# mozack/vdjer

Hardware: NVIDIA B200
Metric: graph_build_prune_windows_per_sec (higher is better)
Workload: dtype u8/u64

## Files before the change

### vdjer_b200/csrc/kernels.cuh

```cuda
#pragma once
#include <cstdint>
#include <cuda_runtime.h>

namespace vdjg {

typedef unsigned long long u64;
typedef unsigned int u32;
typedef unsigned short u16;
typedef unsigned char u8;

constexpr u64 EMPTY64 = ~0ull;
constexpr u64 INF64 = ~0ull;
constexpr u32 NIL32 = 0xFFFFFFFFu;
constexpr u32 CNT_CAP = 32765;
constexpr int GATE_Q = 20;
constexpr int HIQ = 30;
constexpr int FLB = 6;
constexpr u32 CNT2_MASK = 0x00FFFFFFu;
constexpr int CNT2_IN = 24;
constexpr u64 LOG_A = 1ull << 62, LOG_B = 1ull << 63;
constexpr int QSUM_SAT = 214;
constexpr int MAX_LOG_RANKS = 11;
constexpr u32 CNT_MULTI = 0x80000000u;
constexpr u32 CNT_SURV = 0x40000000u;
// ... 294 lines not shown
            if (rev && code < 4) code = 3u - code;
            const u8 q = (u8)(rec[1 + g.L + sj] - '!');
            a.qual[r * (u64)g.L + j] = q;
            okq = q >= GATE_Q;
            hiq = q >= HIQ;
        }
        const u32 b0 = __ballot_sync(0xFFFFFFFFu, code < 4 && (code & 1u));
        const u32 b1 = __ballot_sync(0xFFFFFFFFu, code < 4 && (code & 2u));
        const u32 bv = __ballot_sync(0xFFFFFFFFu, code < 4);
        const u32 bg = __ballot_sync(0xFFFFFFFFu, code < 4 && okq);
        const u32 bh = __ballot_sync(0xFFFFFFFFu, code < 4 && hiq);
        const u32 be = __ballot_sync(0xFFFFFFFFu, code == 5);
        if (lane == 0) {
            if (be) atomicMin(&a.bad[1], r);
            a.bases[r * (u64)g.nb + (j0 >> 5)] = spread_bits(b0) | (spread_bits(b1) << 1);
            if (j0 & 32) {
                a.valid[r * (u64)g.nm + (j0 >> 6)] = vword | ((u64)bv << 32);
                a.good[r * (u64)g.nm + (j0 >> 6)] = gword | ((u64)bg << 32);
                a.hiq[r * (u64)g.nm + (j0 >> 6)] = hword | ((u64)bh << 32);
            } else {
                vword = bv; gword = bg; hword = bh;
                if (j0 + 32 >= g.L) {
                    a.valid[r * (u64)g.nm + (j0 >> 6)] = vword;
                    a.good[r * (u64)g.nm + (j0 >> 6)] = gword;
                    a.hiq[r * (u64)g.nm + (j0 >> 6)] = hword;
                }
            }
        }
    }
}
__global__ void __launch_bounds__(THREADS)
k_pack(PackArgs a, Geom g) {
    const u32 lane = threadIdx.x & 31;
    const u64 warp = ((u64)blockIdx.x * THREADS + threadIdx.x) >> 5, n_warps = ((u64)gridDim.x * THREADS) >> 5;
    const u64 rec_len = 2ull * g.L + 1;
    for (u64 i = warp; i < a.n; i += n_warps) {
        const unsigned char *rec = a.text + i * rec_len;
        if (!a.fwd_only) {
            pack_record(a, g, rec, a.r0 + i, false, lane);
        } else {
            pack_record(a, g, rec, a.r0 + 2 * i, false, lane);
            pack_record(a, g, rec, a.r0 + 2 * i + 1, true, lane);
        }
    }
}

struct BlockTiles {
    u64 *buf;
    u64 *bar;
    u32 words, off_b, off_c, off_d;
    __device__ __forceinline__ const u64 *a(int i) const { return buf + i * words; }
    __device__ __forceinline__ const u64 *b(int i) const { return buf + i * words + off_b; }
    __device__ __forceinline__ const u64 *c(int i) const { return buf + i * words + off_c; }
    __device__ __forceinline__ const u64 *d(int i) const { return buf + i * words + off_d; }
};
__host__ __device__ inline size_t block_tile_bytes(const Geom &g, int n_masks) {
    return (size_t)2 * g.tile_rec * (size_t)(g.nb + n_masks * g.nm) * 8 + 16;
}
__device__ __forceinline__ BlockTiles tiles_setup(unsigned char *smem, const Geom &g, int n_masks) {
    BlockTiles t;
    t.words = g.tile_rec * (u32)(g.nb + n_masks * g.nm);
    t.off_b = g.tile_rec * (u32)g.nb;
    t.off_c = t.off_b + g.tile_rec * (u32)g.nm;
    t.off_d = t.off_c + g.tile_rec * (u32)g.nm;
    t.buf = reinterpret_cast<u64 *>(smem);
    t.bar = t.buf + 2 * t.words;
    if (threadIdx.x == 0) {
        mbar_init(&t.bar[0], 1);
        mbar_init(&t.bar[1], 1);
        fence_mbar_init();
        fence_proxy_async();
    }
    __syncthreads();
    return t;
}
__device__ __forceinline__ void tiles_issue(const BlockTiles &t, int i, const Geom &g, u64 tile,
                                            const u64 *ga, const u64 *gb, const u64 *gc, const u64 *gd = nullptr) {
    const u32 bytes_a = g.tile_rec * (u32)g.nb * 8u, bytes_m = g.tile_rec * (u32)g.nm * 8u;
    u64 *dst = t.buf + i * t.words;
    mbar_expect_tx(&t.bar[i], bytes_a + (gd ? 3 : 2) * bytes_m);
    tma_load_1d(dst, ga + tile * g.tile_rec * (u64)g.nb, bytes_a, &t.bar[i]);
    tma_load_1d(dst + t.off_b, gb + tile * g.tile_rec * (u64)g.nm, bytes_m, &t.bar[i]);
    tma_load_1d(dst + t.off_c, gc + tile * g.tile_rec * (u64)g.nm, bytes_m, &t.bar[i]);
    if (gd) tma_load_1d(dst + t.off_d, gd + tile * g.tile_rec * (u64)g.nm, bytes_m, &t.bar[i]);
}

__device__ __forceinline__ void extract_bits128(const u64 *m, int nw, int bit0, u64 &lo, u64 &hi) {
    const int wi = bit0 >> 6, sh = bit0 & 63;
    const u64 w0 = wi < nw ? m[wi] : 0ull;
    const u64 w1 = wi + 1 < nw ? m[wi + 1] : 0ull;
    const u64 w2 = wi + 2 < nw ? m[wi + 2] : 0ull;
    if (sh) { lo = (w0 >> sh) | (w1 << (64 - sh)); hi = (w1 >> sh) | (w2 << (64 - sh)); }
    else { lo = w0; hi = w1; }
}
__device__ __forceinline__ void shr128(u64 &lo, u64 &hi, int s) {
    if (s >= 64) { lo = hi >> (s - 64); hi = 0ull; }
    else if (s) { lo = (lo >> s) | (hi << (64 - s)); hi >>= s; }
}
__device__ __forceinline__ u64 erode128(u64 lo, u64 hi, int k) {
    u64 pl = lo, ph = hi, al = ~0ull, ah = ~0ull;
    int alen = 0;
    for (int plen = 1; plen <= k; plen <<= 1) {
        if (k & plen) {
            u64 tl = pl, th = ph;
            shr128(tl, th, alen);
            al &= tl; ah &= th;
            alen += plen;
        }
        u64 tl = pl, th = ph;
        shr128(tl, th, plen);
        pl &= tl; ph &= th;
    }
    return al;
}
__device__ __forceinline__ u64 erode64(u64 m, int k) {
    u64 p = m, a = ~0ull;
    int alen = 0;
    for (int plen = 1; plen <= k; plen <<= 1) {
        if (k & plen) { a &= p >> alen; alen += plen; }
        p &= p >> plen;
    }
    return a;
}
__device__ __forceinline__ u64 window_mask(const u64 *m, int nw, int i0, const Geom &g) {
    u64 lo, hi;
    extract_bits128(m, nw, i0, lo, hi);
    return g.seg + g.k <= 64 ? erode64(lo, g.k) : erode128(lo, hi, g.k);
}

struct Mini {
    u32 *buf;
    u32 x, pre;
    int r;
    __device__ __forceinline__ void sweep(int span) {
        u32 run = ~0u;
        for (int j = span - 1; j >= 0; j--) { run = min(run, buf[j * THREADS]); buf[j * THREADS] = run; }
    }
    __device__ __forceinline__ u32 start(u64 lo, u64 hi, const Geom &g) {
        for (int j = 0; j < g.span; j++) {
            x = (u32)lo & g.mmask;
            buf[j * THREADS] = mini_hash(x);
            lo = (lo >> 2) | (hi << 62);
            hi >>= 2;
        }
        sweep(g.span);
        r = 0; pre = ~0u;
        return buf[0];
    }
    __device__ __forceinline__ u32 step(u32 c, const Geom &g) {
        x = (x >> 2) | (c << (2 * (g.m - 1)));
        const u32 h = mini_hash(x);
        buf[r * THREADS] = h;
        r++;
        if (r == g.span) { sweep(g.span); r = 0; pre = ~0u; return buf[0]; }
        pre = min(pre, h);
        return min(buf[r * THREADS], pre);
    }
};

struct SegRuns {
    u64 V, G, H;
    u32 starts;
    u32 left;
    u32 ord;
    __device__ __forceinline__ bool next(int n, int &s, int &len) {
        if (!left) return false;
        s = __ffs((int)left) - 1;
        left &= left - 1;
        const u64 stop = ((((u64)starts | ~V) >> s) >> 1) | (1ull << (n - s - 1));
        len = __ffsll((long long)stop);
        ord++;
        return true;
    }
    __device__ __forceinline__ u32 has_next(int s, int len) const { return (u32)(V >> (s + len)) & 1u; }
};
template <bool KMERS, class OnGated>
__device__ __forceinline__ SegRuns scan_runs(const u64 *sb, const u64 *sg, const u64 *sv, const u64 *sh, u32 rec, int i0, int n,
                                             const Geom &g, u32 *scratch, u8 *sbk, OnGated on_gated) {
    Mini mn;
    mn.buf = scratch;
    SegRuns sr;
    sr.V = sr.G = sr.H = 0; sr.starts = 0; sr.ord = 0;
    u64 lo = 0, hi = 0, nbase = 0;
    if (n > 0) {
        sr.V = window_mask(sv + (size_t)rec * g.nm, g.nm, i0, g);
        sr.G = window_mask(sg + (size_t)rec * g.nm, g.nm, i0, g);
        if (sh) sr.H = window_mask(sh + (size_t)rec * g.nm, g.nm, i0, g);
        const u64 *b = sb + (size_t)rec * g.nb;
        extract_kmer(b, g.nb, i0, g.kmask_lo, g.kmask_hi, lo, hi);
        const int j = i0 + g.k;
        u64 nl = 0, nh;
        if (j < 32 * g.nb) extract_kmer(b, g.nb, j, ~0ull, 0ull, nl, nh);
        nbase = nl;
    }
    u32 run_len = 0, run_b = 0, minh = 0, n_starts = 0;
    for (int j = 0; j < g.seg; j++) {
        if (j < n) {
            if (j == 0) minh = mn.start(lo, hi, g);
            else {
                const u32 c = (u32)nbase & 3u;
                nbase >>= 2;
                minh = mn.step(c, g);
                if (KMERS) kmer_succ(lo, hi, c, g.k, lo, hi);
            }
            const bool v = (sr.V >> j) & 1ull;
            const u32 b = mini_bucket(minh);
            const bool fresh = v && (run_len == 0 || b != run_b || run_len == (u32)g.run_max);
            if (fresh) {
                sbk[n_starts * THREADS] = (u8)b;
                n_starts++;
                sr.starts |= 1u << j;
                run_b = b;
                run_len = 0;
            }
            run_len = v ? run_len + 1 : 0;
            if (KMERS && ((sr.G >> j) & 1ull)) on_gated(lo, hi, b);
        }
    }
    sr.left = sr.starts;
    return sr;
}

__host__ __device__ inline size_t align128(size_t x) { return (x + 127) & ~(size_t)127; }
__host__ __device__ inline size_t count_head_bytes() {
    return ((size_t)NBUCKET * BHLL / 4 + (size_t)3 * NBUCKET) * sizeof(u32);
}
__host__ __device__ inline size_t scratch_bytes(const Geom &g) { return (size_t)g.span * THREADS * sizeof(u32); }
__host__ __device__ inline size_t sbk_bytes(const Geom &g) { return align128((size_t)g.seg * THREADS); }
__device__ __forceinline__ void byte_max(u32 *words, u32 idx, u32 v, bool global) {
    u32 *wp = words + (idx >> 2);
    const u32 sh = (idx & 3u) * 8u;
    u32 cur = *reinterpret_cast<volatile u32 *>(wp);
    while (((cur >> sh) & 0xFFu) < v) {
        const u32 nv = (cur & ~(0xFFu << sh)) | (v << sh);
        const u32 old = atomicCAS(wp, cur, nv);
        if (old == cur) break;
        cur = old;
    }
}
__global__ void __launch_bounds__(THREADS)
k_count(const u64 *__restrict__ bases, const u64 *__restrict__ good, const u64 *__restrict__ valid,
        Geom g, u64 tile0, u64 tile1 , u32 *hll, u64 *hist ) {
    extern __shared__ __align__(128) unsigned char smem[];
    constexpr int HW = NBUCKET * BHLL / 4;
    u32 *reg = reinterpret_cast<u32 *>(smem);
    u32 *sh = reg + HW;
    for (int i = threadIdx.x; i < HW + 3 * NBUCKET; i += THREADS) reg[i] = 0;
    u32 *scratch = reinterpret_cast<u32 *>(smem + count_head_bytes()) + threadIdx.x;
    u8 *sbk = smem + count_head_bytes() + scratch_bytes(g) + threadIdx.x;
    BlockTiles t = tiles_setup(smem + count_head_bytes() + scratch_bytes(g) + sbk_bytes(g), g, 2);
    const u32 rec = threadIdx.x / (u32)g.segs, i0 = (threadIdx.x % (u32)g.segs) * (u32)g.seg;
    const int n = rec < g.tile_rec ? max(0, min(g.seg, g.w - (int)i0)) : 0;
    const u64 n_iter = (tile1 - tile0 + gridDim.x - 1) / gridDim.x;
    if (threadIdx.x == 0 && tile0 + blockIdx.x < tile1) tiles_issue(t, 0, g, tile0 + blockIdx.x, bases, good, valid);
    u64 tile = tile0 + blockIdx.x;
    for (u64 it = 0; it < n_iter; it++, tile += gridDim.x) {
        const int buf = (int)(it & 1);
        if (tile < tile1) {
            if (threadIdx.x == 0 && tile + gridDim.x < tile1) tiles_issue(t, buf ^ 1, g, tile + gridDim.x, bases, good, valid);
            mbar_wait(&t.bar[buf], (u32)(it >> 1) & 1);
            SegRuns sr = scan_runs<true>(t.a(buf), t.b(buf), t.c(buf), nullptr, rec, (int)i0, n, g, scratch, sbk,
                [&](u64 lo, u64 hi, u32 b) {
                    const u64 h = hash_key(lo, hi);
                    byte_max(reg, b * BHLL + ((u32)h & (BHLL - 1)), (u32)__clzll((long long)(h >> BHLL_BITS)) - (BHLL_BITS - 1), false);
                });
            int rs, len;
            while (sr.next(n, rs, len)) {
                const u32 b = sbk[(sr.ord - 1) * THREADS], gm = (u32)(sr.G >> rs) & ((1u << len) - 1u);
                atomicAdd(&sh[b], 1u);
                if (gm) atomicAdd(&sh[NBUCKET + b], (u32)__popc(gm));
                atomicAdd(&sh[2 * NBUCKET + b], (u32)len);
            }
        }
        __syncthreads();
        if ((it & 0xFFFF) == 0xFFFF) {
            for (int i = threadIdx.x; i < 3 * NBUCKET; i += THREADS) { u32 v = sh[i]; if (v) { atomicAdd(&hist[i], (u64)v); sh[i] = 0; } }
            __syncthreads();
        }
    }
    for (int i = threadIdx.x; i < HW; i += THREADS) {
        const u32 v = reg[i];
        for (int b = 0; v && b < 4; b++) if ((v >> (8 * b)) & 0xFFu) byte_max(hll, 4u * i + b, (v >> (8 * b)) & 0xFFu, true);
    }
    for (int i = threadIdx.x; i < 3 * NBUCKET; i += THREADS)
        if (sh[i]) atomicAdd(&hist[i], (u64)sh[i]);
}

constexpr int RUN_WORDS = 4;
constexpr int RUN_FP_BITS = 22;
__device__ __forceinline__ u32 run_len(u64 w2) { return ((u32)(w2 >> 48) & 31u) + 1u; }
__device__ __forceinline__ u32 run_bucket(u64 w3) { return (u32)(w3 >> STAMP_BITS) & (NBUCKET - 1); }
__device__ __forceinline__ void ld_run(const u64 *p, u64 &a, u64 &b, u64 &c, u64 &d) {
    asm volatile("ld.global.cs.v4.b64 {%0,%1,%2,%3}, [%4];" : "=l"(a), "=l"(b), "=l"(c), "=l"(d) : "l"(p) : "memory");
}

struct ScatterArgs {
    const u64 *bases, *good, *valid, *hiq;
    u64 *const *tbase;
    u64 *cursor;
    const u64 *limit;
    u64 rec_base;
    Counters *ctr;
};
struct ScatterSmem {
    u32 *cnt;
    u32 *fill;
    u32 *boff;
    u64 *gbase;
    u64 **dst;
    u32 *fp;
    u32 *n_list;
    u8 *sbk;
    u64 *list;
    u64 *stage;
    unsigned char *tiles;
};
__host__ __device__ inline size_t scatter_carve(ScatterSmem *o, unsigned char *base, const Geom &g) {
    size_t off = 0;
    auto take = [&](size_t bytes) { size_t at = off; off = align128(off + bytes); return at; };
    const size_t a_cnt = take((size_t)NBUCKET * 4), a_fill = take((size_t)NBUCKET * 4), a_boff = take((size_t)(NBUCKET + 1) * 4), a_gbase = take((size_t)NBUCKET * 8);
    const size_t a_dst = take((size_t)NBUCKET * 8), a_fp = take((size_t)g.tile_rec * 4), a_n = take(16);
    const size_t a_list = take((size_t)g.stage_runs * 16), a_sbk = take(sbk_bytes(g));
    const size_t stage_b = (size_t)g.stage_runs * RUN_WORDS * 8, scr_b = scratch_bytes(g);
    const size_t a_stage = take(stage_b > scr_b ? stage_b : scr_b), a_tiles = take(block_tile_bytes(g, 3));
    if (o) {
        o->cnt = reinterpret_cast<u32 *>(base + a_cnt); o->fill = reinterpret_cast<u32 *>(base + a_fill); o->boff = reinterpret_cast<u32 *>(base + a_boff);
        o->gbase = reinterpret_cast<u64 *>(base + a_gbase); o->dst = reinterpret_cast<u64 **>(base + a_dst);
        o->fp = reinterpret_cast<u32 *>(base + a_fp); o->n_list = reinterpret_cast<u32 *>(base + a_n);
        o->sbk = base + a_sbk;
        o->list = reinterpret_cast<u64 *>(base + a_list); o->stage = reinterpret_cast<u64 *>(base + a_stage);
        o->tiles = base + a_tiles;
    }
    return off;
}
__device__ __forceinline__ void build_run(u64 d0, u64 d1, const u64 *sb, const u64 *sv, const u32 *sfp, const Geom &g, u64 rec0,
                                          u64 &w0, u64 &w1, u64 &w2, u64 &w3) {
    const u32 rec = (u32)d1 & 0xFFFFu, a = (u32)(d1 >> 16) & 0xFFu, b = (u32)(d1 >> 24) & 0xFFu;
    extract_kmer(sb + (size_t)rec * g.nb, g.nb, (int)a, ~0ull, ~0ull, w0, w1);
    const u32 f = sfp[rec], fp = f & ((1u << RUN_FP_BITS) - 1);
    u64 prev = 0;
    if (a > 0 && bit_at(sv + (size_t)rec * g.nm, (int)a - 1)) prev = 1ull | ((u64)base_at(sb + (size_t)rec * g.nb, (int)a - 1) << 1);
    w2 = d0 | ((u64)(f >> 31) << 54) | (prev << 55) | ((u64)(fp >> 16) << 58);
    w3 = ((rec0 + rec) * (u64)g.w + a) | ((u64)b << STAMP_BITS) | ((u64)(fp & 0xFFFFu) << 48);
}

__global__ void __launch_bounds__(THREADS)
k_scatter(ScatterArgs a, Geom g, Part pt) {
    extern __shared__ __align__(128) unsigned char smem[];
    const int NU = NBUCKET >> pt.ushift;
    ScatterSmem sm;
    scatter_carve(&sm, smem, g);
    BlockTiles t = tiles_setup(sm.tiles, g, 3);
    const u32 lane = threadIdx.x & 31, wid = threadIdx.x >> 5;
    u32 *scratch = reinterpret_cast<u32 *>(sm.stage) + threadIdx.x;
    const u32 rec = threadIdx.x / (u32)g.segs, i0 = (threadIdx.x % (u32)g.segs) * (u32)g.seg;
    const int n = rec < g.tile_rec ? max(0, min(g.seg, g.w - (int)i0)) : 0;
    const u64 n_iter = (g.n_tiles + gridDim.x - 1) / gridDim.x;
    for (int u = threadIdx.x; u < NU; u += THREADS) sm.dst[u] = a.tbase[u];
    if (threadIdx.x == 0 && blockIdx.x < g.n_tiles) tiles_issue(t, 0, g, blockIdx.x, a.bases, a.good, a.valid, a.hiq);
    u64 tile = blockIdx.x;
    for (u64 it = 0; it < n_iter; it++, tile += gridDim.x) {
        const int buf = (int)(it & 1);
        if (tile >= g.n_tiles) break;
        for (int i = threadIdx.x; i < NU; i += THREADS) { sm.cnt[i] = 0; sm.fill[i] = 0; }
        if (threadIdx.x == 0) {
            *sm.n_list = 0;
            if (tile + gridDim.x < g.n_tiles) tiles_issue(t, buf ^ 1, g, tile + gridDim.x, a.bases, a.good, a.valid, a.hiq);
        }
        mbar_wait(&t.bar[buf], (u32)(it >> 1) & 1);
        __syncthreads();
        const u64 *sb = t.a(buf), *sg = t.b(buf), *sv = t.c(buf), *sh = t.d(buf);
        const u64 rec0 = a.rec_base + tile * g.tile_rec;
        for (u32 r = threadIdx.x; r < g.tile_rec; r += THREADS) {
            u64 h = 0x9E3779B97F4A7C15ull;
            for (int i = 0; i < g.nb; i++) h = hash_key(sb[(size_t)r * g.nb + i], h);
            for (int i = 0; i < g.nm; i++) h = hash_key(sv[(size_t)r * g.nm + i], h);
            const u32 rec_hi = (extract_mask(sh + (size_t)r * g.nm, g.nm, 0) & g.kones) == g.kones ? 1u : 0u;
            sm.fp[r] = ((u32)(h >> 32) & ((1u << RUN_FP_BITS) - 1)) | (rec_hi << 31);
        }
        __syncthreads();
        {
            SegRuns sr = scan_runs<false>(sb, sg, sv, sh, rec, (int)i0, n, g, scratch, sm.sbk + threadIdx.x, [](u64, u64, u32) {});
            for (;;) {
                int rs = 0, len = 1;
                const bool has = sr.next(n, rs, len);
                if (!__ballot_sync(0xFFFFFFFFu, has)) break;
                const u32 b = has ? sm.sbk[(sr.ord - 1) * THREADS + threadIdx.x] : 0u, u = b >> pt.ushift;
                const bool ship = has && sm.dst[u];
                const u32 ball = __ballot_sync(0xFFFFFFFFu, ship);
                if (!ball) continue;
                u32 e0 = 0;
                if (lane == 0) e0 = atomicAdd(sm.n_list, (u32)__popc(ball));
                e0 = __shfl_sync(0xFFFFFFFFu, e0, 0);
                if (ship) {
                    const u32 lm = (1u << len) - 1u;
                    const u64 d0 = (u64)((u32)(sr.G >> rs) & lm) | ((u64)((u32)(sr.H >> rs) & lm) << 24) | ((u64)(len - 1) << 48) |
                                   ((u64)sr.has_next(rs, len) << 53);
                    const u64 d1 = (u64)rec | ((u64)(i0 + rs) << 16) | ((u64)b << 24);
                    const u32 e = e0 + (u32)__popc(ball & ((1u << lane) - 1u));
                    if (e < g.stage_runs) {
                        sm.list[2 * e] = d0; sm.list[2 * e + 1] = d1;
                        atomicAdd(&sm.cnt[u], 1u);
                    } else {
                        u64 w0, w1, w2, w3;
                        build_run(d0, d1, sb, sv, sm.fp, g, rec0, w0, w1, w2, w3);
                        const u64 at = atomicAdd(&a.cursor[u], 1ull);
                        if (at < a.limit[u]) st_sector(sm.dst[u] + at * RUN_WORDS, w0, w1, w2, w3);
                        else atomicExch(&a.ctr->overflow, 4u);
                    }
                }
            }
        }
        __syncthreads();
        for (int u = threadIdx.x; u < NU; u += THREADS) {
            const u32 c = sm.cnt[u];
            u64 gbs = INF64;
            if (c) {
                gbs = atomicAdd(&a.cursor[u], (u64)c);
                if (gbs + c > a.limit[u]) { atomicExch(&a.ctr->overflow, 4u); gbs = INF64; }
            }
            sm.gbase[u] = gbs;
        }
        if (wid == 0) {
            const int per = (NU + 31) / 32;
            u32 sum = 0;
            for (int j = 0; j < per; j++) { int u = lane * per + j; if (u < NU) sum += sm.cnt[u]; }
            u32 incl = sum;
            for (int o = 1; o < 32; o <<= 1) { u32 v = __shfl_up_sync(0xFFFFFFFFu, incl, o); if ((int)lane >= o) incl += v; }
            u32 run = incl - sum;
            for (int j = 0; j < per; j++) {
                int u = lane * per + j;
                if (u < NU) { sm.boff[u] = run; run += sm.cnt[u]; }
            }
            if (lane == 31) sm.boff[NU] = run;
        }
        __syncthreads();
        const u32 n_list = min(*sm.n_list, g.stage_runs);
        for (u32 e = threadIdx.x; e < n_list; e += THREADS) {
            const u64 d0 = sm.list[2 * e], d1 = sm.list[2 * e + 1];
            const u32 u = ((u32)(d1 >> 24) & 0xFFu) >> pt.ushift;
            u64 w0, w1, w2, w3;
            build_run(d0, d1, sb, sv, sm.fp, g, rec0, w0, w1, w2, w3);
            u64 *dst = sm.stage + (size_t)(sm.boff[u] + atomicAdd(&sm.fill[u], 1u)) * RUN_WORDS;
            dst[0] = w0; dst[1] = w1; dst[2] = w2; dst[3] = w3;
        }
        fence_proxy_async();
        __syncthreads();
        for (int u = threadIdx.x; u < NU; u += THREADS) {
            const u32 c = sm.boff[u + 1] - sm.boff[u];
            const u64 gbs = sm.gbase[u];
            if (c && gbs != INF64) tma_store_1d(sm.dst[u] + gbs * RUN_WORDS, sm.stage + (size_t)sm.boff[u] * RUN_WORDS, c * (u32)(RUN_WORDS * 8));
        }
        tma_store_commit();
        tma_store_wait_read();
        __syncthreads();
    }
}

__global__ void k_init_table1(Slot1 *t, u64 cap) {
    u64 i = (u64)blockIdx.x * blockDim.x + threadIdx.x, stride = (u64)gridDim.x * blockDim.x;
    for (; i < cap; i += stride)
        st_sector(&t[i], EMPTY64, EMPTY64, (u64)0 | ((u64)NIL32 << 32), (u64)NIL32);
}
__global__ void k_init_table2(Slot2 *t, u64 cap) {
    u64 i = (u64)blockIdx.x * blockDim.x + threadIdx.x, stride = (u64)gridDim.x * blockDim.x;
    for (; i < cap; i += stride) {
        st_sector(&t[i], EMPTY64, EMPTY64, (u64)0 | ((u64)NIL32 << 32), INF64);
        st_sector(reinterpret_cast<char *>(&t[i]) + 32, INF64, INF64, INF64, INF64);
    }
}

__device__ __noinline__ bool same_words(const u64 *b1, const u64 *b2, int nb, const u64 *v1, const u64 *v2, int nm) {
    u64 diff = 0;
    for (int i = 0; i < nb; i++) diff |= b1[i] ^ b2[i];
    for (int i = 0; i < nm; i++) diff |= v1[i] ^ v2[i];
    return diff == 0;
}
__device__ __forceinline__ bool same_read(const Reads &rd, u64 r1, u64 r2, int nb, int nm) {
    const int d1 = rd.dev_of(r1), d2 = rd.dev_of(r2);
    const u64 l1 = r1 - rd.rec_base[d1], l2 = r2 - rd.rec_base[d2];
    if (rd.any_strand && rd.strand[d1][l1] != rd.strand[d2][l2]) return false;
    return same_words(rd.bases[d1] + l1 * nb, rd.bases[d2] + l2 * nb, nb, rd.valid[d1] + l1 * nm, rd.valid[d2] + l2 * nm, nm);
}

struct Pass1Args {
    const u64 *runs;
    Reads rd;
    Slot1 *table;
    u64 cap;
    u64 *log;
    u32 log_blocks;
    u32 nb_ranks;
    Counters *ctr;
};

constexpr u32 QFLUSH = 96;
constexpr u32 QCAP = 32 * BATCH + QFLUSH;
constexpr u32 QDENSE = 20;
constexpr int HOTC_BITS = 6;
constexpr u32 HOTC = 1u << HOTC_BITS;
constexpr u32 QFLUSH1 = 32;
constexpr u32 QCAP1 = 32 * BATCH + QFLUSH1;
template <bool WIDE, u32 QC = QCAP>
struct WarpQueue {
    u64 *lo, *w1, *w2;
    u32 *idx;
    __device__ __forceinline__ void setup(unsigned char *smem) {
        unsigned char *p = smem + (threadIdx.x >> 5) * bytes();
        lo = reinterpret_cast<u64 *>(p);
        w1 = lo + QC;
        w2 = w1 + QC;
        idx = reinterpret_cast<u32 *>(w1 + (WIDE ? 2 : 1) * QC);
    }
    __host__ __device__ static constexpr size_t bytes() { return (size_t)QC * (WIDE ? 28 : 20); }
    template <class Make>
    __device__ __forceinline__ u32 push_lazy(u32 qn, bool defer, u64 l, u32 i, Make make) {
        const u32 lane = threadIdx.x & 31;
        const u32 ballot = __ballot_sync(0xFFFFFFFFu, defer);
        if (defer) {
            const u32 pos = qn + __popc(ballot & ((1u << lane) - 1));
            u64 a, b;
            make(a, b);
            lo[pos] = l; w1[pos] = a; idx[pos] = i;
            if (WIDE) w2[pos] = b;
        }
        return qn + __popc(ballot);
    }
    __device__ __forceinline__ u32 push(u32 qn, bool defer, u64 l, u64 a, u64 b, u32 i) {
        const u32 lane = threadIdx.x & 31;
        const u32 ballot = __ballot_sync(0xFFFFFFFFu, defer);
        if (defer) {
            const u32 pos = qn + __popc(ballot & ((1u << lane) - 1));
            lo[pos] = l; w1[pos] = a; idx[pos] = i;
            if (WIDE) w2[pos] = b;
        }
        return qn + __popc(ballot);
    }
};

struct RunCursor {
    u64 w0, w1, w2;
    u64 stamp0;
    u32 off, len;
    u32 l;
    u32 j;
    u32 rem;
};
struct RunFeed {
    u64 *rw;
    u32 cnt, incl, total;
    u32 live;
    template <bool GATED_ONLY>
    __device__ __forceinline__ static u32 selected(u64 w2) {
        return GATED_ONLY ? (u32)w2 & 0xFFFFFFu : (1u << run_len(w2)) - 1u;
    }
    template <bool GATED_ONLY>
    __device__ __forceinline__ void load(const u64 *runs, u64 ri, u64 n_runs) {
        const u32 lane = threadIdx.x & 31;
        u64 w0 = 0, w1 = 0, w2 = 0, w3 = 0;
        cnt = 0;
        if (ri < n_runs) {
            ld_run(runs + ri * RUN_WORDS, w0, w1, w2, w3);
            cnt = (u32)__popc(selected<GATED_ONLY>(w2));
        }
        incl = cnt;
        for (int o = 1; o < 32; o <<= 1) { const u32 v = __shfl_up_sync(0xFFFFFFFFu, incl, o); if ((int)lane >= o) incl += v; }
        total = __shfl_sync(0xFFFFFFFFu, incl, 31);
        live = __ballot_sync(0xFFFFFFFFu, cnt != 0);
        __syncwarp();
        u64 *p = rw + lane * RUN_WORDS;
        p[0] = w0; p[1] = w1; p[2] = ri < n_runs ? w2 : 0ull; p[3] = w3;
        __syncwarp();
    }
    template <bool TAB2>
    __device__ __forceinline__ void open(RunCursor &c, const Part &pt) const {
        const u64 *p = rw + c.l * RUN_WORDS;
        c.w0 = p[0]; c.w1 = p[1]; c.w2 = p[2];
        const u64 w3 = p[3];
        c.stamp0 = w3 & ((1ull << STAMP_BITS) - 1);
        const uint4 ut = __ldg(reinterpret_cast<const uint4 *>(pt.ut + (run_bucket(w3) >> pt.ushift)));
        c.off = TAB2 ? ut.z : ut.x;
        c.len = TAB2 ? ut.w : ut.y;
    }
    template <bool GATED_ONLY, bool TAB2>
    __device__ __forceinline__ void seek(u32 t, RunCursor &c, const Part &pt) const {
        u32 l = 0;
#pragma unroll
        for (int s = 16; s; s >>= 1) { const u32 v = __shfl_sync(0xFFFFFFFFu, incl, l + s - 1); if (v <= t) l += s; }
        u32 nth = t - __shfl_sync(0xFFFFFFFFu, incl - cnt, l);
        c.l = l;
        open<TAB2>(c, pt);
        u32 m = selected<GATED_ONLY>(c.w2), j = 0;
        if (GATED_ONLY) {
#pragma unroll
            for (int s = 16; s; s >>= 1) {
                const u32 k = (u32)__popc(m & ((1u << s) - 1u));
                if (nth >= k) { nth -= k; m >>= s; j += s; }
            }
            m >>= 1;
        } else {
            j = nth;
            m >>= j + 1;
        }
        c.j = j; c.rem = m;
    }
    __device__ __forceinline__ u32 fingerprint(u32 l, const Part &pt) const {
        const u64 *p = rw + l * RUN_WORDS;
        return (((u32)(p[3] >> 48) & 0xFFFFu) | (((u32)(p[2] >> 58) & 0x3Fu) << 16)) & (u32)((1ull << pt.fb) - 1);
    }
    template <bool GATED_ONLY, bool TAB2>
    __device__ __forceinline__ void next(RunCursor &c, const Part &pt) const {
        if (c.rem) {
            const u32 s = (u32)__ffs((int)c.rem);
            c.j += s; c.rem >>= s;
            return;
        }
        const u32 ahead = c.l < 31 ? live >> (c.l + 1) : 0u;
        c.l += ahead ? (u32)__ffs((int)ahead) : 0u;
        open<TAB2>(c, pt);
        const u32 m = selected<GATED_ONLY>(c.w2);
        const u32 s = m ? (u32)__ffs((int)m) : 1u;
        c.j = s - 1; c.rem = m >> s;
    }
};
__device__ __forceinline__ void run_kmer(const Geom &g, const RunCursor &c, u64 &lo, u64 &hi, u32 &idx) {
    const u32 sh = 2u * c.j;
    lo = sh ? (c.w0 >> sh) | (c.w1 << (64 - sh)) : c.w0;
    hi = c.w1 >> sh;
    lo &= g.kmask_lo; hi &= g.kmask_hi;
    idx = slot_in(hash_slot(lo, hi), c.off, c.len);
}
__device__ __forceinline__ u32 run_flags(const Geom &g, u64 w0, u64 w1, u64 w2, u32 j) {
    const u32 p = j + (u32)g.k;
    const u32 nb = (u32)((p < 32 ? w0 >> (2 * p) : w1 >> (2 * (p - 32)))) & 3u;
    const bool has_next = j + 1 < run_len(w2) || ((w2 >> 53) & 1ull);
    return (has_next ? 1u | (nb << 1) : 0u) | ((u32)(w2 >> (24 + j)) & 1u) << 3 | ((u32)(w2 >> 54) & 1u) << 4;
}
__device__ __forceinline__ u32 run_flags2(const Geom &g, u64 w0, u64 w1, u64 w2, u32 j) {
    const u32 p = j + (u32)g.k;
    const u32 nb = (u32)((p < 32 ? w0 >> (2 * p) : w1 >> (2 * (p - 32)))) & 3u;
    const bool has_next = j + 1 < run_len(w2) || ((w2 >> 53) & 1ull);
    const u32 prev = j ? 1u | (((u32)(w0 >> (2 * (j - 1))) & 3u) << 1) : (u32)(w2 >> 55) & 7u;
    return (has_next ? 1u | (nb << 1) : 0u) | prev << 3;
}
template <bool WIDE>
__device__ __forceinline__ void pack_tuple(const Part &pt, u64 hi, u32 fl, u32 fp, u64 stamp, u64 &t1, u64 &t2) {
    t1 = hi | ((u64)fl << pt.hb) | ((u64)fp << (pt.hb + FLB));
    if (WIDE) t2 = stamp;
    else { t1 |= stamp << (pt.hb + FLB + pt.fb); t2 = 0; }
}

struct LogCursor { u32 base, used; };

template <bool WIDE>
__device__ __forceinline__ u32 pass1_drain(const Pass1Args &a, const Geom &g, const Part &pt, WarpQueue<WIDE, QCAP1> &q,
                                           u32 qn, LogCursor &lc, bool final) {
    const u32 lane = threadIdx.x & 31, lt = (1u << lane) - 1;
    u32 next = 0;
    bool have = false;
    u64 lo = 0, hi = 0, stamp = 0, rw1 = 0, rw2 = 0;
    u32 idx = 0, probe = 0, fp = 0, fl = 0;
    __syncwarp();
    for (;;) {
        const u32 need = __ballot_sync(0xFFFFFFFFu, !have);
        const u32 avail = qn - next;
        if (avail == 0 && (need == 0xFFFFFFFFu || (!final && 32 - __popc(need) < (int)pt.qdense1))) break;
        if (need && avail) {
            const u32 my = __popc(need & lt);
            if (!have && my < avail) {
                const u32 e = next + my;
                lo = q.lo[e]; rw1 = q.w1[e]; rw2 = WIDE ? q.w2[e] : 0ull;
                tuple_decode<WIDE>(pt, rw1, rw2, hi, fl, fp, stamp);
                idx = q.idx[e];
                probe = 0;
                have = true;
            }
            next += min((u32)__popc(need), avail);
        }
        bool found = false, claimed = false;
        u64 q2 = 0, q3 = 0;
        Slot1 *slot = a.table + idx;
        if (have) {
            u64 q0, q1;
            ld_sector(slot, q0, q1, q2, q3);
            if (q0 == EMPTY64 && q1 == EMPTY64) {
                cas128(slot, EMPTY64, EMPTY64, lo, hi, q0, q1);
                if (q0 == EMPTY64 && q1 == EMPTY64) { found = claimed = true; q2 = (u64)NIL32 << 32; q3 = (u64)NIL32; }
                else if (q0 == lo && q1 == hi) q2 = (u64)NIL32 << 32;
            } else if (q0 == lo && q1 == hi) {
                found = (u32)q3 != NIL32 && (a.nb_ranks == 0 || (u32)(q2 >> 32) != NIL32);
            }
            if (!found && !(q0 == lo && q1 == hi)) {
                if (++idx == (u32)a.cap) idx = 0;
                if (++probe >= MAX_PROBE) { atomicExch(&a.ctr->overflow, 1u); have = false; }
            }
        }
        u32 blk = (u32)(q2 >> 32);
        if (a.nb_ranks) {
            const u32 ballot = __ballot_sync(0xFFFFFFFFu, claimed);
            if (ballot) {
                const u32 n = __popc(ballot), room = LOG_CHUNK - lc.used, my = __popc(ballot & lt);
                u32 fresh = 0;
                if (n > room) {
                    if (lane == 0) fresh = atomicAdd(&a.ctr->log_used, LOG_CHUNK);
                    fresh = __shfl_sync(0xFFFFFFFFu, fresh, 0);
                }
                if (claimed) {
                    blk = my < room ? lc.base + lc.used + my : fresh + (my - room);
                    if (blk < a.log_blocks) slot->head = blk;
                    else { atomicExch(&a.ctr->overflow, 2u); blk = NIL32; slot->head = 0; }
                }
                if (n > room) { lc.base = fresh; lc.used = n - room; }
                else lc.used += n;
            }
        }
        if (found) {
            const u32 r = g.w_magic ? (u32)__umul64hi(stamp, g.w_magic) : (u32)stamp;
            const u64 entry = stamp | ((fl & 8u) ? LOG_A : 0ull) | ((fl & 16u) ? LOG_B : 0ull);
            if (claimed) {
                if (a.nb_ranks && blk != NIL32) a.log[(u64)blk * a.nb_ranks] = entry;
                st_cg_u64(reinterpret_cast<u64 *>(&slot->first_rec), (u64)r | ((u64)fp << 32));
            } else {
                const u32 cw = (u32)q2, cnt = cw & CNT_MASK;
                const u32 first_rec = (u32)q3, first_fp = (u32)(q3 >> 32);
                u32 rank = NIL32;
                if (cnt + 1 < a.nb_ranks) rank = (atomicAdd(&slot->count, 1u) & CNT_MASK) + 1;
                else if (cnt + 1 < CNT_CAP) atomicAdd(&slot->count, 1u);
                if (!(cw & CNT_MULTI) && first_rec != r &&
                    (first_fp != fp || !same_read(a.rd, first_rec, r, g.nb, g.nm)))
                    atomicOr(&slot->count, CNT_MULTI);
                if (rank < a.nb_ranks && blk != NIL32) a.log[(u64)blk * a.nb_ranks + rank] = entry;
            }
            have = false;
        }
    }
    __syncwarp();
    const u32 left = q.push(0, have, lo, rw1, rw2, idx);
    __syncwarp();
    return left;
}

__device__ __forceinline__ void hot_flush(Slot1 *table, u32 *hidx, u32 *hcnt) {
    for (u32 i = threadIdx.x & 31; i < HOTC; i += 32) {
        const u32 c = hcnt[i];
        if (c) {
            u32 *cp = &table[hidx[i]].count;
            if ((*reinterpret_cast<volatile u32 *>(cp) & CNT_MASK) < (1u << 24)) atomicAdd(cp, c);
        }
        hidx[i] = NIL32; hcnt[i] = 0;
    }
}

template <bool WIDE>
__global__ void __launch_bounds__(THREADS, PASS1_MIN_BLOCKS)
k_pass1(Pass1Args a, Geom g, Part pt) {
    extern __shared__ __align__(128) unsigned char smem[];
// ... 878 lines not shown
```

Baseline: 21.88 billion.

## Fuse record fingerprint into scan and keep bucket reservations in registers

Each thread now computes its record fingerprint inline before scanning runs, instead of a separate per-tile fingerprint loop followed by a block barrier. Per-bucket cursor reservations are kept in thread registers rather than a shared gbase array, which drops that array from shared memory, and counter resets move to the end of each iteration so two __syncthreads per tile go away. The trade-off is that every segment thread of a record recomputes the same hash, and overflow checking now happens at store time.

```diff
diff --git a/profiles/scatter_occupancy.cu b/profiles/scatter_occupancy.cu
--- /dev/null
+++ b/profiles/scatter_occupancy.cu
@@ -0,0 +1,16 @@
+#include "vdjgraph.cu"
+
+int main(int argc, char **argv) {
+    vdjgraph_ctx c;
+    c.prm.read_length = argc > 1 ? atoi(argv[1]) : 50;
+    c.prm.kmer_size = argc > 2 ? atoi(argv[2]) : 35;
+    make_geom(&c, 1);
+    const size_t smem = scatter_carve(nullptr, nullptr, c.g);
+    const int bps = blocks_per_sm((const void *)k_scatter, smem);
+    cudaFuncAttributes fa = {};
+    const cudaError_t e = cudaFuncGetAttributes(&fa, (const void *)k_scatter);
+    printf("k_scatter L=%d k=%d: stage %u runs, %zu bytes of shared memory per block, %d registers, %d blocks per SM%s\n",
+           c.prm.read_length, c.prm.kmer_size, c.g.stage_runs, smem, fa.numRegs, bps,
+           e == cudaSuccess ? "" : " (no device: not measured)");
+    return e == cudaSuccess ? 0 : 1;
+}
diff --git a/vdjer_b200/csrc/kernels.cuh b/vdjer_b200/csrc/kernels.cuh
--- a/vdjer_b200/csrc/kernels.cuh
+++ b/vdjer_b200/csrc/kernels.cuh
@@ -620,11 +620,11 @@
     u64 rec_base;
     Counters *ctr;
 };
+static_assert(NBUCKET <= THREADS, "k_scatter: thread u reserves and stores unit u");
 struct ScatterSmem {
     u32 *cnt;
     u32 *fill;
     u32 *boff;
-    u64 *gbase;
     u64 **dst;
     u32 *fp;
     u32 *n_list;
@@ -636,14 +636,14 @@
 __host__ __device__ inline size_t scatter_carve(ScatterSmem *o, unsigned char *base, const Geom &g) {
     size_t off = 0;
     auto take = [&](size_t bytes) { size_t at = off; off = align128(off + bytes); return at; };
-    const size_t a_cnt = take((size_t)NBUCKET * 4), a_fill = take((size_t)NBUCKET * 4), a_boff = take((size_t)(NBUCKET + 1) * 4), a_gbase = take((size_t)NBUCKET * 8);
+    const size_t a_cnt = take((size_t)NBUCKET * 4), a_fill = take((size_t)NBUCKET * 4), a_boff = take((size_t)(NBUCKET + 1) * 4);
     const size_t a_dst = take((size_t)NBUCKET * 8), a_fp = take((size_t)g.tile_rec * 4), a_n = take(16);
     const size_t a_list = take((size_t)g.stage_runs * 16), a_sbk = take(sbk_bytes(g));
     const size_t stage_b = (size_t)g.stage_runs * RUN_WORDS * 8, scr_b = scratch_bytes(g);
     const size_t a_stage = take(stage_b > scr_b ? stage_b : scr_b), a_tiles = take(block_tile_bytes(g, 3));
     if (o) {
         o->cnt = reinterpret_cast<u32 *>(base + a_cnt); o->fill = reinterpret_cast<u32 *>(base + a_fill); o->boff = reinterpret_cast<u32 *>(base + a_boff);
-        o->gbase = reinterpret_cast<u64 *>(base + a_gbase); o->dst = reinterpret_cast<u64 **>(base + a_dst);
+        o->dst = reinterpret_cast<u64 **>(base + a_dst);
         o->fp = reinterpret_cast<u32 *>(base + a_fp); o->n_list = reinterpret_cast<u32 *>(base + a_n);
         o->sbk = base + a_sbk;
         o->list = reinterpret_cast<u64 *>(base + a_list); o->stage = reinterpret_cast<u64 *>(base + a_stage);
@@ -651,11 +651,18 @@
     }
     return off;
 }
-__device__ __forceinline__ void build_run(u64 d0, u64 d1, const u64 *sb, const u64 *sv, const u32 *sfp, const Geom &g, u64 rec0,
+__device__ __forceinline__ u32 record_fp(const u64 *sb, const u64 *sv, const u64 *sh, u32 r, const Geom &g) {
+    u64 h = 0x9E3779B97F4A7C15ull;
+    for (int i = 0; i < g.nb; i++) h = hash_key(sb[(size_t)r * g.nb + i], h);
+    for (int i = 0; i < g.nm; i++) h = hash_key(sv[(size_t)r * g.nm + i], h);
+    const u32 rec_hi = (extract_mask(sh + (size_t)r * g.nm, g.nm, 0) & g.kones) == g.kones ? 1u : 0u;
+    return ((u32)(h >> 32) & ((1u << RUN_FP_BITS) - 1)) | (rec_hi << 31);
+}
+__device__ __forceinline__ void build_run(u64 d0, u64 d1, const u64 *sb, const u64 *sv, u32 f, const Geom &g, u64 rec0,
                                           u64 &w0, u64 &w1, u64 &w2, u64 &w3) {
     const u32 rec = (u32)d1 & 0xFFFFu, a = (u32)(d1 >> 16) & 0xFFu, b = (u32)(d1 >> 24) & 0xFFu;
     extract_kmer(sb + (size_t)rec * g.nb, g.nb, (int)a, ~0ull, ~0ull, w0, w1);
-    const u32 f = sfp[rec], fp = f & ((1u << RUN_FP_BITS) - 1);
+    const u32 fp = f & ((1u << RUN_FP_BITS) - 1);
     u64 prev = 0;
     if (a > 0 && bit_at(sv + (size_t)rec * g.nm, (int)a - 1)) prev = 1ull | ((u64)base_at(sb + (size_t)rec * g.nb, (int)a - 1) << 1);
     w2 = d0 | ((u64)(f >> 31) << 54) | (prev << 55) | ((u64)(fp >> 16) << 58);
@@ -674,30 +681,22 @@
     const u32 rec = threadIdx.x / (u32)g.segs, i0 = (threadIdx.x % (u32)g.segs) * (u32)g.seg;
     const int n = rec < g.tile_rec ? max(0, min(g.seg, g.w - (int)i0)) : 0;
     const u64 n_iter = (g.n_tiles + gridDim.x - 1) / gridDim.x;
-    for (int u = threadIdx.x; u < NU; u += THREADS) sm.dst[u] = a.tbase[u];
+    for (int u = threadIdx.x; u < NU; u += THREADS) { sm.dst[u] = a.tbase[u]; sm.cnt[u] = 0; sm.fill[u] = 0; }
+    if (threadIdx.x == 0) *sm.n_list = 0;
+    __syncthreads();
+    const u64 ulim = threadIdx.x < NU ? a.limit[threadIdx.x] : 0ull;
     if (threadIdx.x == 0 && blockIdx.x < g.n_tiles) tiles_issue(t, 0, g, blockIdx.x, a.bases, a.good, a.valid, a.hiq);
     u64 tile = blockIdx.x;
     for (u64 it = 0; it < n_iter; it++, tile += gridDim.x) {
         const int buf = (int)(it & 1);
         if (tile >= g.n_tiles) break;
-        for (int i = threadIdx.x; i < NU; i += THREADS) { sm.cnt[i] = 0; sm.fill[i] = 0; }
-        if (threadIdx.x == 0) {
-            *sm.n_list = 0;
-            if (tile + gridDim.x < g.n_tiles) tiles_issue(t, buf ^ 1, g, tile + gridDim.x, a.bases, a.good, a.valid, a.hiq);
-        }
+        if (threadIdx.x == 0 && tile + gridDim.x < g.n_tiles) tiles_issue(t, buf ^ 1, g, tile + gridDim.x, a.bases, a.good, a.valid, a.hiq);
         mbar_wait(&t.bar[buf], (u32)(it >> 1) & 1);
-        __syncthreads();
         const u64 *sb = t.a(buf), *sg = t.b(buf), *sv = t.c(buf), *sh = t.d(buf);
         const u64 rec0 = a.rec_base + tile * g.tile_rec;
-        for (u32 r = threadIdx.x; r < g.tile_rec; r += THREADS) {
-            u64 h = 0x9E3779B97F4A7C15ull;
-            for (int i = 0; i < g.nb; i++) h = hash_key(sb[(size_t)r * g.nb + i], h);
-            for (int i = 0; i < g.nm; i++) h = hash_key(sv[(size_t)r * g.nm + i], h);
-            const u32 rec_hi = (extract_mask(sh + (size_t)r * g.nm, g.nm, 0) & g.kones) == g.kones ? 1u : 0u;
-            sm.fp[r] = ((u32)(h >> 32) & ((1u << RUN_FP_BITS) - 1)) | (rec_hi << 31);
-        }
-        __syncthreads();
         {
+            const u32 fp = n > 0 ? record_fp(sb, sv, sh, rec, g) : 0u;
+            if (n > 0 && i0 == 0) sm.fp[rec] = fp;
             SegRuns sr = scan_runs<false>(sb, sg, sv, sh, rec, (int)i0, n, g, scratch, sm.sbk + threadIdx.x, [](u64, u64, u32) {});
             for (;;) {
                 int rs = 0, len = 1;
@@ -721,7 +720,7 @@
                         atomicAdd(&sm.cnt[u], 1u);
                     } else {
                         u64 w0, w1, w2, w3;
-                        build_run(d0, d1, sb, sv, sm.fp, g, rec0, w0, w1, w2, w3);
+                        build_run(d0, d1, sb, sv, fp, g, rec0, w0, w1, w2, w3);
                         const u64 at = atomicAdd(&a.cursor[u], 1ull);
                         if (at < a.limit[u]) st_sector(sm.dst[u] + at * RUN_WORDS, w0, w1, w2, w3);
                         else atomicExch(&a.ctr->overflow, 4u);
@@ -730,15 +729,9 @@
             }
         }
         __syncthreads();
-        for (int u = threadIdx.x; u < NU; u += THREADS) {
-            const u32 c = sm.cnt[u];
-            u64 gbs = INF64;
-            if (c) {
-                gbs = atomicAdd(&a.cursor[u], (u64)c);
-                if (gbs + c > a.limit[u]) { atomicExch(&a.ctr->overflow, 4u); gbs = INF64; }
-            }
-            sm.gbase[u] = gbs;
-        }
+        const u32 c = threadIdx.x < NU ? sm.cnt[threadIdx.x] : 0u;
+        u64 gbs = 0;
+        if (c) gbs = atomicAdd(&a.cursor[threadIdx.x], (u64)c);
         if (wid == 0) {
             const int per = (NU + 31) / 32;
             u32 sum = 0;
@@ -758,18 +751,19 @@
             const u64 d0 = sm.list[2 * e], d1 = sm.list[2 * e + 1];
             const u32 u = ((u32)(d1 >> 24) & 0xFFu) >> pt.ushift;
             u64 w0, w1, w2, w3;
-            build_run(d0, d1, sb, sv, sm.fp, g, rec0, w0, w1, w2, w3);
+            build_run(d0, d1, sb, sv, sm.fp[(u32)d1 & 0xFFFFu], g, rec0, w0, w1, w2, w3);
             u64 *dst = sm.stage + (size_t)(sm.boff[u] + atomicAdd(&sm.fill[u], 1u)) * RUN_WORDS;
             dst[0] = w0; dst[1] = w1; dst[2] = w2; dst[3] = w3;
         }
         fence_proxy_async();
         __syncthreads();
-        for (int u = threadIdx.x; u < NU; u += THREADS) {
-            const u32 c = sm.boff[u + 1] - sm.boff[u];
-            const u64 gbs = sm.gbase[u];
-            if (c && gbs != INF64) tma_store_1d(sm.dst[u] + gbs * RUN_WORDS, sm.stage + (size_t)sm.boff[u] * RUN_WORDS, c * (u32)(RUN_WORDS * 8));
-        }
-        tma_store_commit();
+        if (c) {
+            if (gbs + c > ulim) atomicExch(&a.ctr->overflow, 4u);
+            else tma_store_1d(sm.dst[threadIdx.x] + gbs * RUN_WORDS, sm.stage + (size_t)sm.boff[threadIdx.x] * RUN_WORDS, c * (u32)(RUN_WORDS * 8));
+            tma_store_commit();
+        }
+        if (threadIdx.x < NU) { sm.cnt[threadIdx.x] = 0; sm.fill[threadIdx.x] = 0; }
+        if (threadIdx.x == 0) *sm.n_list = 0;
         tma_store_wait_read();
         __syncthreads();
     }
```

Result: no change. 21.99 billion (median of 6 runs) (+0.5%).
